# rbesenczi/newMSM

Hardware: AMD Instinct MI355X
Metric: label-cost evals/sec (higher is better)
Workload: dtype f64; 1 GPU; pairwise sulc (D=1) unary label-cost table, ico6 data grid / ico4 control grid, 19 labels, 48678 evals = 3187573 point samples per step (BASELINE config 2); kind=univariate, simmeasure=correlation, replicas=1

## Files before the change

include/msmhip.h:

```cpp
#ifndef MSMHIP_H
#define MSMHIP_H

#include <stddef.h>
#include <stdint.h>

#ifdef __cplusplus
extern "C" {
#endif

#define MSM_ABI_VERSION 11

#define MSM_OK 0
#define MSM_ERR_INVALID (-1)
#define MSM_ERR_HIP (-2)
#define MSM_ERR_OUTSIDE (-3)
#define MSM_ERR_NOTFOUND (-4)
#define MSM_ERR_NOGPU (-5)
#define MSM_ERR_STATE (-6)
#define MSM_ERR_CAPACITY (-7)
#define MSM_ERR_ROTATION (-8)

#define MSM_RAD 100.0
#define MSM_FOLDING 1e7

typedef struct msm_ctx msm_ctx;
typedef struct msm_mesh msm_mesh;
typedef struct msm_cost msm_cost;

int         msm_abi_version(void);
const char *msm_last_error(void);
int         msm_device_count(void);

int msm_icosphere_counts(int order, int32_t *V, int32_t *T);
int msm_icosphere(int order, double radius, double *xyz, int32_t *tri);
int msm_mesh_adjacency(const int32_t *tri, int32_t V, int32_t T, int32_t *nbr_ptr, int32_t *nbr, int32_t *tid_ptr, int32_t *tid);
int msm_vertex_areas(const double *xyz, const int32_t *tri, int32_t V, int32_t T, double *area);
int msm_resample_anatomy_grid(const double *cp_xyz, int32_t N, const int32_t *cp_tri, int32_t Tc, int32_t levels, double rad, int32_t *Va, int32_t *Ta,
                              double *axyz, int32_t *atri, int32_t *w_ptr, int32_t *w_cp, double *w_val, int32_t *face_ptr, int32_t *face_idx);
int msm_cp_spacings(const double *xyz, const int32_t *tri, int32_t V, int32_t T, double *maxsep, double *mvdmax);
int msm_label_sampling_grid(int sg_order, double max_dist, int abs_is_int, int32_t cap,
                            double *samples, int32_t *nsamples, double *barycentres, int32_t *nbarycentres);
int msm_rescale_sampling_grid(const double *samples, int32_t n, double *scale, double *labels);
int msm_rotation_matrix(const double ci[3], const double index[3], double R[9]);
int msm_cp_rotations(const double centre[3], const double *cp_xyz, int32_t N, double *rot);
int msm_estimate_triplets(const int32_t *tri, int32_t T, int32_t *triplets);
int msm_estimate_pairs(const int32_t *tri, int32_t V, int32_t T, int32_t *pairs);
int msm_octree_signature(const double *xyz, const int32_t *tri, int32_t V, int32_t T, int64_t stats[5], uint64_t *signature);
int msm_ray_table_check(const double *xyz, const int32_t *tri, int32_t V, int32_t T, int32_t nsamples, uint64_t seed, int64_t report[10]);

msm_ctx *msm_ctx_create(int device);
msm_ctx *msm_ctx_create_on_stream(int device, void *hip_stream);
void     msm_ctx_destroy(msm_ctx *ctx);
int      msm_ctx_synchronize(msm_ctx *ctx);
void    *msm_ctx_stream(msm_ctx *ctx);
void     msm_store_release_i64(int64_t *addr, int64_t value);
int64_t  msm_load_acquire_i64(const int64_t *addr);
int64_t  msm_min_acquire_i64(const int64_t *addr, int32_t n);
int      msm_ctx_wait_stream(msm_ctx *ctx, void *hip_stream);
int      msm_ctx_staging_stats(msm_ctx *ctx, int64_t out[4]);
int      msm_ctx_time_queries(msm_ctx *ctx, int enable);
int      msm_ctx_query_kernel_ms(msm_ctx *ctx, double *ms);
int      msm_query_lanes(int64_t n_queries);
void    *msm_host_alloc(msm_ctx *ctx, size_t bytes);
void     msm_host_free(msm_ctx *ctx, void *p);
int      msm_host_register(msm_ctx *ctx, void *p, size_t bytes);

msm_mesh *msm_mesh_create(msm_ctx *ctx, const double *xyz, int32_t V, const int32_t *tri, int32_t T);
void      msm_mesh_destroy(msm_mesh *m);
int       msm_mesh_update_coords(msm_mesh *m, const double *xyz);
int       msm_mesh_get_coords(msm_mesh *m, double *xyz);
int       msm_mesh_set_features(msm_mesh *m, const double *feat, int32_t D);
int       msm_mesh_sizes(const msm_mesh *m, int32_t *V, int32_t *T, int32_t *D);
int       msm_mesh_octree_stats(msm_mesh *m, int64_t stats[5]);
int       msm_mesh_octree_signature(msm_mesh *m, int64_t stats[5], uint64_t *signature);
int       msm_octree_forest_signatures(msm_ctx *ctx, const double *xyz, int32_t V, const int32_t *tri, int32_t T, int32_t B, uint64_t *signatures);
int       msm_mesh_prepare_search(msm_mesh *m, int wait, int32_t *ready);

#define MSM_WEIGHTS_PROJECTED 0
#define MSM_WEIGHTS_RAW 1
int msm_query_triangles(msm_mesh *target, const double *q_xyz, int32_t N, int32_t *tri_id, int32_t *v_id, double *w, int weight_mode);
int msm_closest_vertex(msm_mesh *target, const double *q_xyz, int32_t N, int32_t *v_id);
int msm_adaptive_barycentric_weights(msm_mesh *in_mesh, msm_mesh *new_mesh, const double *excl,
                                     int32_t *row_ptr, int32_t *col, double *val, int64_t cap, int64_t *nnz);
int msm_metric_resample(msm_mesh *in_mesh, const double *data, int32_t D, msm_mesh *new_mesh, const double *excl, double *out, double *excl_out);
int msm_sphere_project_warp(msm_mesh *from, const double *to_xyz, double *sphere_xyz, int32_t N);
int msm_mesh_sphere_project_warp(msm_mesh *sphere, msm_mesh *from, const double *to_xyz);
int msm_barycentric_coords_resample(msm_mesh *from, const double *coords_xyz, const double *q_xyz, int32_t N, double *out_xyz);
int msm_smooth_data(msm_mesh *orig, const double *data, int32_t D, msm_mesh *sphlow, double sigma, const double *excl, double *out, double *excl_out);
int msm_nearest_neighbour(msm_mesh *orig, const double *data, int32_t D, const double *q_xyz, int32_t N, const double *excl, double *out, double *excl_out);
int msm_create_exclusion(const double *data, int32_t D, int32_t V, double thrl, double thru, double *excl);

int msm_mesh_unfold(msm_mesh *m, double radius, int32_t *passes, int32_t *first_folded);
int msm_variance_normalise(double *data, int32_t D, int32_t V, const double *excl);
int msm_histogram_match(msm_ctx *ctx, int32_t n_src, int32_t D, int32_t Vs, const double *src, const double *src_excl, int32_t src_excl_rows,
                        int32_t Vt, const double *ref, const double *ref_excl, int32_t ref_excl_rows, double *out);
int msm_mcmc_optimise(const double *unary, const double *tcosts, const int32_t *triplets, int32_t N, int32_t L, int32_t T, double mcparam,
                      int32_t iters, uint64_t seed, int32_t *labeling);
int msm_fusion_icm_step(const double *unary2 , const double *quads , const int32_t *pairs , int32_t P,
                        const double *octets , const int32_t *triplets , int32_t T, int32_t N, int32_t max_passes,
                        int32_t *x );
int msm_pairwise_icm(const double *unary, const double *paircosts, const int32_t *pairs, int32_t N, int32_t L, int32_t P, int32_t max_passes, int32_t *labeling);
// ... 134 lines not shown
```

newmsm_amd/_lib.py:

```python
import ctypes as C
import os

_HERE = os.path.dirname(os.path.abspath(__file__))
LIB_PATH = os.environ.get("MSM_LIB_PATH") or os.path.join(_HERE, "libmsmhip.so")

c_dp = C.POINTER(C.c_double)
c_ip = C.POINTER(C.c_int32)
c_lp = C.POINTER(C.c_int64)

MSM_OK = 0
ERR_NAMES = {-1: "MSM_ERR_INVALID", -2: "MSM_ERR_HIP", -3: "MSM_ERR_OUTSIDE", -4: "MSM_ERR_NOTFOUND", -5: "MSM_ERR_NOGPU",
             -6: "MSM_ERR_STATE", -7: "MSM_ERR_CAPACITY", -8: "MSM_ERR_ROTATION"}


class MsmError(RuntimeError):

    def __init__(self, code, message):
        super().__init__("%s (%d): %s" % (ERR_NAMES.get(code, "MSM_ERR"), code, message))
        self.code = code


class GroupParams(C.Structure):
    _fields_ = [("simmeasure", C.c_int32), ("fixnan", C.c_int32), ("lambda_", C.c_double), ("mu", C.c_double),
                ("kappa", C.c_double), ("k_exp", C.c_double), ("rexp", C.c_double), ("range", C.c_double), ("percentile", C.c_double)]


class CostParams(C.Structure):
    _fields_ = [("kind", C.c_int32), ("simmeasure", C.c_int32), ("rmode", C.c_int32), ("reserved", C.c_int32),
                ("lambda_", C.c_double), ("mu", C.c_double), ("kappa", C.c_double), ("k_exp", C.c_double),
                ("rexp", C.c_double), ("range", C.c_double), ("percentile", C.c_double)]


_VP = C.c_void_p
SIGNATURES = {
    "msm_abi_version": (C.c_int, []),
    "msm_last_error": (C.c_char_p, []),
    "msm_device_count": (C.c_int, []),
    "msm_icosphere_counts": (C.c_int, [C.c_int, c_ip, c_ip]),
    "msm_icosphere": (C.c_int, [C.c_int, C.c_double, c_dp, c_ip]),
    "msm_mesh_adjacency": (C.c_int, [c_ip, C.c_int32, C.c_int32, c_ip, c_ip, c_ip, c_ip]),
    "msm_vertex_areas": (C.c_int, [c_dp, c_ip, C.c_int32, C.c_int32, c_dp]),
    "msm_resample_anatomy_grid": (C.c_int, [c_dp, C.c_int32, c_ip, C.c_int32, C.c_int32, C.c_double, c_ip, c_ip, c_dp, c_ip, c_ip, c_ip, c_dp, c_ip, c_ip]),
    "msm_cp_spacings": (C.c_int, [c_dp, c_ip, C.c_int32, C.c_int32, c_dp, c_dp]),
    "msm_label_sampling_grid": (C.c_int, [C.c_int, C.c_double, C.c_int, C.c_int32, c_dp, c_ip, c_dp, c_ip]),
    "msm_rescale_sampling_grid": (C.c_int, [c_dp, C.c_int32, c_dp, c_dp]),
    "msm_rotation_matrix": (C.c_int, [c_dp, c_dp, c_dp]),
    "msm_cp_rotations": (C.c_int, [c_dp, c_dp, C.c_int32, c_dp]),
    "msm_estimate_triplets": (C.c_int, [c_ip, C.c_int32, c_ip]),
    "msm_estimate_pairs": (C.c_int, [c_ip, C.c_int32, C.c_int32, c_ip]),
    "msm_octree_signature": (C.c_int, [c_dp, c_ip, C.c_int32, C.c_int32, C.POINTER(C.c_int64), C.POINTER(C.c_uint64)]),
    "msm_ray_table_check": (C.c_int, [c_dp, c_ip, C.c_int32, C.c_int32, C.c_int32, C.c_uint64, C.POINTER(C.c_int64)]),
    "msm_ctx_create": (_VP, [C.c_int]),
    "msm_ctx_create_on_stream": (_VP, [C.c_int, _VP]),
    "msm_ctx_destroy": (None, [_VP]),
    "msm_ctx_synchronize": (C.c_int, [_VP]),
    "msm_ctx_stream": (_VP, [_VP]),
    "msm_store_release_i64": (None, [_VP, C.c_int64]),
    "msm_load_acquire_i64": (C.c_int64, [_VP]),
    "msm_min_acquire_i64": (C.c_int64, [_VP, C.c_int32]),
    "msm_ctx_time_queries": (C.c_int, [_VP, C.c_int]),
    "msm_ctx_query_kernel_ms": (C.c_int, [_VP, c_dp]),
    "msm_query_lanes": (C.c_int, [C.c_int64]),
    "msm_group_context": (_VP, [_VP]),
    "msm_ctx_wait_stream": (C.c_int, [_VP, _VP]),
    "msm_ctx_staging_stats": (C.c_int, [_VP, C.POINTER(C.c_int64)]),
    "msm_host_alloc": (_VP, [_VP, C.c_size_t]),
    "msm_host_free": (None, [_VP, _VP]),
    "msm_host_register": (C.c_int, [_VP, _VP, C.c_size_t]),
    "msm_mesh_create": (_VP, [_VP, c_dp, C.c_int32, c_ip, C.c_int32]),
    "msm_mesh_destroy": (None, [_VP]),
    "msm_mesh_update_coords": (C.c_int, [_VP, c_dp]),
    "msm_mesh_get_coords": (C.c_int, [_VP, c_dp]),
    "msm_mesh_set_features": (C.c_int, [_VP, c_dp, C.c_int32]),
    "msm_mesh_sizes": (C.c_int, [_VP, c_ip, c_ip, c_ip]),
    "msm_mesh_octree_stats": (C.c_int, [_VP, c_lp]),
    "msm_mesh_octree_signature": (C.c_int, [_VP, c_lp, C.POINTER(C.c_uint64)]),
    "msm_octree_forest_signatures": (C.c_int, [_VP, c_dp, C.c_int32, c_ip, C.c_int32, C.c_int32, C.POINTER(C.c_uint64)]),
    "msm_query_triangles": (C.c_int, [_VP, c_dp, C.c_int32, c_ip, c_ip, c_dp, C.c_int]),
    "msm_closest_vertex": (C.c_int, [_VP, c_dp, C.c_int32, c_ip]),
    "msm_adaptive_barycentric_weights": (C.c_int, [_VP, _VP, c_dp, c_ip, c_ip, c_dp, C.c_int64, c_lp]),
    "msm_metric_resample": (C.c_int, [_VP, c_dp, C.c_int32, _VP, c_dp, c_dp, c_dp]),
    "msm_create_exclusion": (C.c_int, [c_dp, C.c_int32, C.c_int32, C.c_double, C.c_double, c_dp]),
    "msm_sphere_project_warp": (C.c_int, [_VP, c_dp, c_dp, C.c_int32]),
    "msm_mesh_sphere_project_warp": (C.c_int, [_VP, _VP, c_dp]),
    "msm_barycentric_coords_resample": (C.c_int, [_VP, c_dp, c_dp, C.c_int32, c_dp]),
    "msm_smooth_data": (C.c_int, [_VP, c_dp, C.c_int32, _VP, C.c_double, c_dp, c_dp, c_dp]),
    "msm_mesh_unfold": (C.c_int, [_VP, C.c_double, c_ip, c_ip]),
    "msm_mesh_prepare_search": (C.c_int, [_VP, C.c_int, c_ip]),
    "msm_variance_normalise": (C.c_int, [c_dp, C.c_int32, C.c_int32, c_dp]),
    "msm_histogram_match": (C.c_int, [_VP, C.c_int32, C.c_int32, C.c_int32, c_dp, c_dp, C.c_int32, C.c_int32, c_dp, c_dp, C.c_int32, c_dp]),
    "msm_mcmc_optimise": (C.c_int, [c_dp, c_dp, c_ip, C.c_int32, C.c_int32, C.c_int32, C.c_double, C.c_int32, C.c_uint64, c_ip]),
    "msm_fusion_icm_step": (C.c_int, [c_dp, c_dp, c_ip, C.c_int32, c_dp, c_ip, C.c_int32, C.c_int32, C.c_int32, c_ip]),
    "msm_pairwise_icm": (C.c_int, [c_dp, c_dp, c_ip, C.c_int32, C.c_int32, C.c_int32, C.c_int32, c_ip]),
    "msm_nearest_neighbour": (C.c_int, [_VP, c_dp, C.c_int32, c_dp, C.c_int32, c_dp, c_dp, c_dp]),
    "msm_cost_create": (_VP, [_VP, C.POINTER(CostParams)]),
    "msm_cost_destroy": (None, [_VP]),
    "msm_cost_set_meshes": (C.c_int, [_VP, _VP, _VP, _VP]),
    "msm_cost_set_anatomical": (C.c_int, [_VP, _VP, c_dp, c_dp, C.c_int32, c_ip, C.c_int32, c_ip, c_ip, c_dp, c_ip, c_ip]),
    "msm_cost_reset_source": (C.c_int, [_VP, _VP]),
    "msm_cost_reset_cpgrid": (C.c_int, [_VP, _VP]),
    "msm_cost_set_source_features": (C.c_int, [_VP, c_dp, C.c_int32]),
    "msm_cost_set_cfweight": (C.c_int, [_VP, c_dp, C.c_int32]),
    "msm_cost_set_spacings": (C.c_int, [_VP, c_dp, C.c_double]),
    "msm_cost_set_labels": (C.c_int, [_VP, c_dp, C.c_int32, c_dp]),
# ... 96 lines not shown
```

newmsm_amd/api.py:

```python
import ctypes as C

import numpy as np

from ._lib import CostParams, MsmError, c_dp, c_ip, c_lp, check, lib

WEIGHTS_PROJECTED = 0
WEIGHTS_RAW = 1
KINDS = dict(univariate=0, multivariate=1, patchwise=2, ho_univariate=3, ho_multivariate=4)


def _soa(points):
    a = np.ascontiguousarray(np.asarray(points, dtype=np.float64).reshape(-1, 3).T)
    return a, a.ctypes.data_as(c_dp)


def _aos(soa, n):
    return np.ascontiguousarray(np.asarray(soa).reshape(3, n).T)


def _tri_soa(tri):
    a = np.ascontiguousarray(np.asarray(tri, dtype=np.int32).reshape(-1, 3).T)
    return a, a.ctypes.data_as(c_ip)


# ... 51 lines not shown
    t, pt = _tri_soa(tri)
    ms = np.zeros(x.shape[1])
    mvd = C.c_double()
    check(lib().msm_cp_spacings(px, pt, x.shape[1], t.shape[1], ms.ctypes.data_as(c_dp), C.byref(mvd)))
    return ms, mvd.value


def label_sampling_grid(sg_order, max_dist, abs_is_int=False, cap=4096):
    s = np.zeros((3, cap))
    b = np.zeros((3, cap))
    ns, nb = C.c_int32(), C.c_int32()
    check(lib().msm_label_sampling_grid(sg_order, float(max_dist), int(abs_is_int), cap, s.ctypes.data_as(c_dp), C.byref(ns),
                                        b.ctypes.data_as(c_dp), C.byref(nb)))
    return np.ascontiguousarray(s[:, : ns.value].T), np.ascontiguousarray(b[:, : nb.value].T)


def rescale_sampling_grid(samples, scale):
    s, ps = _soa(samples)
    n = s.shape[1]
    out = np.zeros((3, n))
    sc = C.c_double(scale)
    check(lib().msm_rescale_sampling_grid(ps, n, C.byref(sc), out.ctypes.data_as(c_dp)))
    return np.ascontiguousarray(out.T), sc.value


def estimate_rotation_matrix(ci, index):
    R = np.zeros(9)
    check(lib().msm_rotation_matrix(_d(ci)[1], _d(index)[1], R.ctypes.data_as(c_dp)))
    return R.reshape(3, 3)


def cp_rotations(centre, cp_xyz):
    x, px = _soa(cp_xyz)
    rot = np.zeros((x.shape[1], 9))
    check(lib().msm_cp_rotations(_d(centre)[1], px, x.shape[1], rot.ctypes.data_as(c_dp)))
    return rot


def octree_signature(xyz, tri):
    x, px = _soa(xyz)
    t, pt = _tri_soa(tri)
    stats = (C.c_int64 * 5)()
    sig = C.c_uint64(0)
    check(lib().msm_octree_signature(px, pt, x.shape[1], t.shape[1], stats, C.byref(sig)))
    return dict(nodes=stats[0], leaves=stats[1], depth=stats[2], refs=stats[3], max_leaf=stats[4]), sig.value


def ray_table_check(xyz, tri, nsamples=20000, seed=1):
    x, px = _soa(xyz)
    t, pt = _tri_soa(tri)
    rep = (C.c_int64 * 10)()
    check(lib().msm_ray_table_check(px, pt, x.shape[1], t.shape[1], nsamples, seed, rep))
    return dict(points=rep[0], by_float=rep[1], by_fp64=rep[2], open=rep[3], violations=rep[4], unusable=rep[5], with_exclusions=rep[6], simple=bool(rep[7]), boxes_checked=rep[8], refused_by_boxes=rep[9])


def estimate_triplets(tri):
    t, pt = _tri_soa(tri)
    out = np.zeros((t.shape[1], 3), dtype=np.int32)
    check(lib().msm_estimate_triplets(pt, t.shape[1], out.ctypes.data_as(c_ip)))
    return out


def estimate_pairs(tri, V):
    t, pt = _tri_soa(tri)
    n = lib().msm_estimate_pairs(pt, V, t.shape[1], None)
    if n < 0:
        check(n)
    out = np.zeros((n, 2), dtype=np.int32)
    lib().msm_estimate_pairs(pt, V, t.shape[1], out.ctypes.data_as(c_ip))
    return out


class Context:

    def __init__(self, device=0, stream=None):
        L = lib()
        self.h = L.msm_ctx_create(device) if stream is None else L.msm_ctx_create_on_stream(device, C.c_void_p(stream))
        if not self.h:
            raise MsmError(-5, L.msm_last_error().decode())
        self.device = device

    def synchronize(self):
        check(lib().msm_ctx_synchronize(self.h))

    @property
    def stream(self):
        return lib().msm_ctx_stream(self.h)

    def wait_stream(self, hip_stream=None):
        check(lib().msm_ctx_wait_stream(self.h, C.c_void_p(hip_stream or 0)))

    def staging_stats(self):
        out = (C.c_int64 * 4)()
        check(lib().msm_ctx_staging_stats(self.h, out))
        return dict(blocks=int(out[0]), bytes=int(out[1]), allocated=int(out[2]), waits=int(out[3]))

    def host_array(self, shape, dtype=np.float64):
        n = int(np.prod(shape)) * np.dtype(dtype).itemsize
        p = lib().msm_host_alloc(self.h, max(n, 8))
        if not p:
            raise MsmError(-2, lib().msm_last_error().decode())
        buf = (C.c_char * max(n, 8)).from_address(p)
        return np.frombuffer(buf, dtype=dtype, count=int(np.prod(shape))).reshape(shape)

    def scratch_host_array(self, name, shape, dtype=np.float64):
        n = int(np.prod(shape)) * np.dtype(dtype).itemsize
# ... 767 lines not shown
```

newmsm_amd/csrc/internal.hpp:

```cpp
#pragma once

#include <hip/hip_runtime.h>

#include <cstdarg>
#include <cstdint>
#include <cstdio>
#include <functional>
#include <memory>
#include <mutex>
#include <string>
#include <vector>

#include "../../include/msmhip.h"
#include "devbuf.hpp"
#include "geom.hpp"

namespace msm {

void set_error(const char *fmt, ...);
int fail(int code, const char *fmt, ...);
void pool_trim();
size_t pool_idle_bytes();

#define MSM_HIP(call)                                                                                 \
    do {                                                                                              \
        hipError_t e_ = (call);                                                                       \
        if (e_ != hipSuccess) return msm::fail(MSM_ERR_HIP, "%s failed: %s", #call, hipGetErrorString(e_)); \
    } while (0)

#define MSM_TRY(call)               \
    do {                            \
        const int st_ = (call);     \
        if (st_) return st_;        \
    } while (0)

struct Adjacency {
    std::vector<int32_t> nbr_ptr, nbr, tid_ptr, tid;
};
void build_adjacency(const int32_t *tri , int V, int T, Adjacency &adj);
void icosphere_unit(int order, std::vector<double> &xyz_aos, std::vector<int32_t> &tri_aos);

struct alignas(128) TriRec {
    double v0[3], v1[3], v2[3];
    double s3[3];
    double d;
    int32_t id[3];
    int32_t tri;
    double reserved;
};
static_assert(sizeof(TriRec) == 128, "TriRec must be 128 bytes");

constexpr int kRayPieces = 9;

struct RayTable {
    bool simple = false;
    int G = 0;
    std::vector<int4> cell;
    std::vector<float4> edge;
    std::vector<int4> more;
    std::vector<int4> excl;
    double r2lo = 0, r2hi = 0;
};

struct FlatOctree {
    std::vector<int4> node;
    std::vector<double4> nodebox;
    int nmask_blocks = 0;
    std::vector<int32_t> parent;
    std::vector<int32_t> leaf_tri;
    std::vector<int32_t> grid;
    int grid_depth = 0;
    RayTable rays;
    int64_t stats[5] = {0, 0, 0, 0, 0};
    int dev_nnodes = 0, dev_entries = 0;
    int nnodes() const { return node.empty() ? dev_nnodes : (int)node.size(); }
    int nentries() const { return node.empty() ? dev_entries : (int)leaf_tri.size(); }
};
void build_octree(const double *xyz , const int32_t *tri , int V, int T, FlatOctree &out);
void build_ray_table(const double *xyz, const int32_t *tri, int V, int T, FlatOctree &tree);

struct DevTree {
    const int4 *node;
    const int32_t *parent;
    const int32_t *leaf_tri;
    const float4 *cone;
    const TriRec *rec;
    const int32_t *grid;
    int grid_depth;
    int simple;
    const unsigned long long *mask;
    int nnodes;
    int ray_G;
    const int4 *ray_cell;
    const float4 *ray_tri;
    const int4 *ray_more, *ray_excl;
    double ray_r2lo, ray_r2hi;
};

}

namespace msm {
struct Stager;
}

struct msm_ctx {
// ... 141 lines not shown
```

newmsm_amd/csrc/octree.cpp:

```cpp
#include <algorithm>
#include <atomic>
#include <cmath>
#include <chrono>
#include <cstdio>
#include <cstdlib>
#include <deque>
#include <unordered_map>

#include "host_parallel.hpp"
#include "internal.hpp"
#include "search_device.hpp"

#define TICK(name) do { if (std::getenv("MSMHIP_TIMING")) { auto now_ = std::chrono::steady_clock::now(); fprintf(stderr, "  %s %.1f ms\n", name, std::chrono::duration<double, std::milli>(now_ - tick_).count()); tick_ = now_; } } while (0)

namespace msm {

namespace {

struct BNode {
    int first_child = -1;
    int parent = -1;
    double b[3][3];
    std::vector<int32_t> tris;
    int total_size = 0, num_split = 0;
};

struct Builder {
    const double *xyz;
    const int32_t *tri;
    int V, T;
    std::deque<BNode> nodes;
    std::vector<double> box;
    const double *bxp = nullptr;

    void precompute_boxes() {
        box.resize((size_t)6 * T);
        bxp = box.data();
        parallel_chunks(T, T < 20000 ? 1 : std::min(host_workers(), 8), [&](int, int t0, int t1) {
            for (int t = t0; t < t1; ++t) {
                double *lo = &box[(size_t)6 * t], *hi = lo + 3;
                for (int a = 0; a < 3; ++a) lo[a] = hi[a] = xyz[a * V + tri[t]];
                for (int k = 1; k < 3; ++k)
                    for (int a = 0; a < 3; ++a) {
                        double c = xyz[a * V + tri[k * T + t]];
                        if (c < lo[a]) lo[a] = c;
                        if (c > hi[a]) hi[a] = c;
                    }
            }
        });
    }
    void aabb(int t, double lo[3], double hi[3]) const {
        const double *b = &bxp[(size_t)6 * t];
        for (int a = 0; a < 3; ++a) {
            lo[a] = b[a];
            hi[a] = b[3 + a];
        }
    }
    bool overlaps(int n, const double lo[3], const double hi[3]) const {
// ... 151 lines not shown
                bool opposite = false;
                for (int f = ptr[v]; f < ptr[v + 1]; ++f) opposite = opposite || head[f] == u;
                if (!opposite) ok.store(false, std::memory_order_relaxed);
            }
    });
    if (!ok.load()) return false;
    const long E = (long)3 * T / 2;
    if ((long)V - E + (long)T != 2) return false;
    return std::fabs(solid - 4.0 * M_PI) < 1e-6;
}

std::vector<double> safe_margins(const double *xyz, const int32_t *tri, int V, int T) {
    std::vector<double> band(T), lmax(T), vband(V, 0.0), margin(T);
    for (int t = 0; t < T; ++t) {
        const int id[3] = {tri[t], tri[T + t], tri[2 * T + t]};
        const V3 a = vtx(xyz, V, id[0]), b = vtx(xyz, V, id[1]), c = vtx(xyz, V, id[2]);
        const double la = norm(sub(b, c)), lb = norm(sub(a, c)), lc = norm(sub(a, b));
        const double area = 0.5 * norm(cross(sub(b, a), sub(c, a)));
        lmax[t] = std::fmax(la, std::fmax(lb, lc));
        const double lmin = std::fmin(la, std::fmin(lb, lc));
        band[t] = (area > 0 && lmin > 0) ? 1e-8 / (2 * area * lmin) : HUGE_VAL;
        if (!(band[t] == band[t])) band[t] = HUGE_VAL;
        for (int k = 0; k < 3; ++k) vband[id[k]] = std::fmax(vband[id[k]], band[t]);
    }
    for (int t = 0; t < T; ++t) {
        const double widest = std::fmax(vband[tri[t]], std::fmax(vband[tri[T + t]], vband[tri[2 * T + t]]));
        const double dist = std::fmax(1e-5 * lmax[t], 1e3 * widest);
        margin[t] = (std::isfinite(dist) && dist < 0.05 * lmax[t]) ? dist : HUGE_VAL;
    }
    return margin;
}

bool lacking_leaves(const FlatOctree &o, int n, const double lo[3], const double hi[3], int t, int cap, std::vector<int> &lack) {
    const double4 box = o.nodebox[n];
    const double blo[3] = {box.x, box.y, box.z};
    for (int a = 0; a < 3; ++a)
        if (hi[a] < blo[a] || lo[a] > blo[a] + box.w) return true;
    const int4 nd = o.node[n];
    if (nd.x < 0) {
        const int32_t *first = o.leaf_tri.data() + nd.y, *last = first + (-nd.x - 1);
        if (std::find(first, last, t) != last) return true;
        if ((int)lack.size() >= cap) return false;
        lack.push_back(n);
        return true;
    }
    for (int c = 0; c < 8; ++c)
        if (!lacking_leaves(o, nd.x + c, lo, hi, t, cap, lack)) return false;
    return true;
}

constexpr double kRayShell = 1e-4;
constexpr int kRayExclMax = 7;

}

void build_ray_table(const double *xyz, const int32_t *tri, int V, int T, FlatOctree &out) {
    auto tick_ = std::chrono::steady_clock::now();
    out.rays.G = 0;
    out.rays.cell.clear();
    out.rays.edge.clear();
    out.rays.simple = simple_star_surface(xyz, tri, V, T);
    const char *no_table = std::getenv("MSMHIP_DISABLE_RAYTABLE");
    if (!out.rays.simple || (no_table && no_table[0] == '1')) return;
    TICK("simple");
    const std::vector<double> margin = safe_margins(xyz, tri, V, T);
    TICK("margins");
    out.rays.edge.assign((size_t)3 * T, make_float4(0.f, 0.f, 0.f, 2.f));
    out.rays.excl.clear();
    out.rays.more.clear();
    out.rays.r2lo = (kRad - kRayShell) * (kRad - kRayShell);
    out.rays.r2hi = (kRad + kRayShell) * (kRad + kRayShell);
    std::vector<char> usable(T, 0);
    const int workers = host_workers();
    struct Chunk {
        std::vector<int4> excl;
        std::vector<int> owner;
    };
    std::vector<Chunk> chunk_out(4 * (size_t)workers + 1);
    parallel_chunks(T, workers, [&](int ci, int t_begin, int t_end) {
    std::vector<int> lack;
    Chunk &mine = chunk_out[ci];
    for (int t = t_begin; t < t_end; ++t) {
        const V3 v[3] = {vtx(xyz, V, tri[t]), vtx(xyz, V, tri[T + t]), vtx(xyz, V, tri[2 * T + t])};
        V3 s3;
        double pd;
        plane_of(v[0], v[1], v[2], s3, pd);
        const double rho = std::fabs(pd);
        if (!(margin[t] < HUGE_VAL) || !(rho > 0)) continue;
        const double thr = margin[t] / rho * (1 + 1e-6) + kRayFloatAllowance;
        if (!(thr < 0.1)) continue;
        V3 u[3];
        double cosmax = 1.0;
        bool ok = true;
        for (int k = 0; k < 3; ++k) {
            const double n = norm(v[k]);
            ok = ok && n > 0;
            u[k] = scale(v[k], 1.0 / n);
        }
        if (!ok) continue;
        for (int k = 0; k < 3; ++k) cosmax = std::fmin(cosmax, dot(u[k], u[(k + 1) % 3]));
        if (!(cosmax > 0.5)) continue;
        const double rlo = kRad - kRayShell, rhi = kRad + kRayShell;
        const double sag = rhi * (1 - std::sqrt(cosmax)) * (1 + 1e-9) + 1e-9;
        double lo[3] = {HUGE_VAL, HUGE_VAL, HUGE_VAL}, hi[3] = {-HUGE_VAL, -HUGE_VAL, -HUGE_VAL};
        for (int k = 0; k < 3; ++k) {
            const double c[3] = {u[k].x, u[k].y, u[k].z};
            for (int a = 0; a < 3; ++a) {
                lo[a] = std::fmin(lo[a], std::fmin(rlo * c[a], rhi * c[a]));
                hi[a] = std::fmax(hi[a], std::fmax(rlo * c[a], rhi * c[a]));
            }
        }
        for (int a = 0; a < 3; ++a) {
            lo[a] -= sag;
            hi[a] += sag;
        }
        lack.clear();
// ... 20 lines not shown
                const double4 nb = out.nodebox[lack[j]];
                const int d = out.node[lack[j]].w;
                if (d > 8) {
                    ok = false;
                    break;
                }
                const double size = 2 * kBounds / (double)(1 << d);
                const int ix = (int)std::lround((nb.x + kBounds) / size), iy = (int)std::lround((nb.y + kBounds) / size), iz = (int)std::lround((nb.z + kBounds) / size);
                bx[j] = (d << 24) | (ix << 16) | (iy << 8) | iz;
            }
            if (!ok) continue;
            excl = (int)mine.excl.size();
            mine.excl.push_back(make_int4(bx[0], bx[1], bx[2], (int)lack.size()));
            mine.owner.push_back(t);
            if (lack.size() > 3) {
                mine.excl.push_back(make_int4(bx[3], bx[4], bx[5], bx[6]));
                mine.owner.push_back(-1);
            }
        }
        e[1].w = __builtin_bit_cast(float, (int32_t)excl);
        e[2].w = 0.f;
        for (int k = 0; k < 3; ++k) out.rays.edge[(size_t)3 * t + k] = e[k];
        usable[t] = 1;
    }
    });
    for (const Chunk &c : chunk_out) {
        const int base = (int)out.rays.excl.size();
        for (size_t k = 0; k < c.excl.size(); ++k) {
            out.rays.excl.push_back(c.excl[k]);
            if (c.owner[k] >= 0) out.rays.edge[(size_t)3 * c.owner[k] + 1].w = __builtin_bit_cast(float, (int32_t)(base + (int)k));
        }
    }
    TICK("edges+robust");
    int G = 8;
    while (G < 512 && (double)G * G * 6 < 4.0 * T) G *= 2;
    out.rays.G = G;
    const size_t ncell = (size_t)6 * G * G;
    struct Cand {
        uint32_t cell;
        float score;
        int32_t tri;
    };
    std::vector<std::vector<Cand>> found_by(4 * (size_t)workers + 1);
    std::vector<int32_t> count(ncell + 1, 0);
    const double m = 1e-5;
    parallel_chunks(T, workers, [&](int ci, int t_begin, int t_end) {
    std::vector<Cand> &found = found_by[ci];
    found.reserve((size_t)(t_end - t_begin) * 8);
    for (int t = t_begin; t < t_end; ++t) {
        if (!usable[t]) continue;
        const V3 v[3] = {vtx(xyz, V, tri[t]), vtx(xyz, V, tri[T + t]), vtx(xyz, V, tri[2 * T + t])};
        const double ln[3] = {norm(v[0]), norm(v[1]), norm(v[2])};
        for (int f = 0; f < 6; ++f) {
            const int a = f >> 1, bb = (a + 1) % 3, cc = (a + 2) % 3;
            const double sgn = (f & 1) ? -1.0 : 1.0;
            double pu[3], pv[3];
            bool front = true;
            for (int k = 0; k < 3; ++k) {
                const double c[3] = {v[k].x, v[k].y, v[k].z};
                const double w = sgn * c[a];
                if (!(w > 0.05 * ln[k])) {
                    front = false;
                    break;
                }
                pu[k] = c[bb] / w;
                pv[k] = c[cc] / w;
            }
            if (!front) continue;
            const double umin = std::fmin(pu[0], std::fmin(pu[1], pu[2])) - m, umax = std::fmax(pu[0], std::fmax(pu[1], pu[2])) + m;
            const double vmin = std::fmin(pv[0], std::fmin(pv[1], pv[2])) - m, vmax = std::fmax(pv[0], std::fmax(pv[1], pv[2])) + m;
            if (umax < -1 || umin > 1 || vmax < -1 || vmin > 1) continue;
            auto cellof = [&](double x) { return std::max(0, std::min(G - 1, (int)std::floor((x + 1) * 0.5 * G))); };
            const int iu0 = cellof(umin), iu1 = cellof(umax), iv0 = cellof(vmin), iv1 = cellof(vmax);
            const double gu = (pu[0] + pu[1] + pu[2]) / 3, gv = (pv[0] + pv[1] + pv[2]) / 3;
            double ex[3], ey[3], ox[3], oy[3], sg[3];
            for (int k = 0; k < 3; ++k) {
                const int p = (k + 1) % 3, q = (k + 2) % 3;
                ex[k] = pu[q] - pu[p], ey[k] = pv[q] - pv[p], ox[k] = pu[p], oy[k] = pv[p];
                sg[k] = (ex[k] * (pv[k] - oy[k]) - ey[k] * (pu[k] - ox[k])) >= 0 ? 1.0 : -1.0;
            }
            for (int iu = iu0; iu <= iu1; ++iu)
                for (int iv = iv0; iv <= iv1; ++iv) {
                    const double x0 = -1 + 2.0 * iu / G - m, x1 = -1 + 2.0 * (iu + 1) / G + m;
                    const double y0 = -1 + 2.0 * iv / G - m, y1 = -1 + 2.0 * (iv + 1) / G + m;
                    bool sep = false;
                    for (int k = 0; k < 3 && !sep; ++k) {
                        auto E = [&](double x, double y) { return sg[k] * (ex[k] * (y - oy[k]) - ey[k] * (x - ox[k])); };
                        sep = E(x0, y0) < 0 && E(x1, y0) < 0 && E(x0, y1) < 0 && E(x1, y1) < 0;
                    }
                    if (sep) continue;
                    const double cu = 0.5 * (x0 + x1) - gu, cv = 0.5 * (y0 + y1) - gv;
                    const size_t cell = ((size_t)f * G + iu) * G + iv;
                    found.push_back(Cand{(uint32_t)cell, (float)(cu * cu + cv * cv), t});
                }
        }
    }
    });
    size_t nfound = 0;
    for (const auto &f : found_by) {
        nfound += f.size();
        for (const Cand &c : f) ++count[c.cell + 1];
    }
    TICK("raster");
    for (size_t c = 0; c < ncell; ++c) count[c + 1] += count[c];
    std::vector<Cand> cand(nfound);
    {
        std::vector<int32_t> fill(count.begin(), count.end() - 1);
        for (const auto &f : found_by)
            for (const Cand &c : f) cand[(size_t)fill[c.cell]++] = c;
    }
    TICK("bucket");
    out.rays.cell.assign(ncell, make_int4(-1, -1, -1, -1));
    parallel_chunks((int)ncell, workers, [&](int, int c_begin, int c_end) {
        for (int c = c_begin; c < c_end; ++c)
            std::sort(cand.data() + count[c], cand.data() + count[c + 1],
                      [](const Cand &x, const Cand &y) { return x.score < y.score || (x.score == y.score && x.tri < y.tri); });
    });
    for (size_t c = 0; c < ncell; ++c) {
        const Cand *first = cand.data() + count[c], *last = cand.data() + count[c + 1];
        int32_t *slot = &out.rays.cell[c].x;
        const int ncand = (int)(last - first);
        if (ncand <= 4) {
            for (int k = 0; k < ncand; ++k) slot[k] = first[k].tri;
        } else {
            for (int k = 0; k < 3; ++k) slot[k] = first[k].tri;
            slot[3] = -2 - (int)out.rays.more.size();
            int4 more = make_int4(-1, -1, -1, -1);
            int32_t *ms = &more.x;
            for (int k = 0; k < 4 && 3 + k < ncand; ++k) ms[k] = first[3 + k].tri;
            out.rays.more.push_back(more);
        }
    }
    TICK("cells");
}

namespace {

void build_top_down(Builder &b) {
    auto tick_ = std::chrono::steady_clock::now();
    std::vector<int32_t> all(b.T);
    for (int t = 0; t < b.T; ++t) all[t] = t;
    const int workers = host_workers();
    if (workers == 1 || b.T < 20000) {
        b.build_down(0, all);
        return;
    }
    struct Job {
        int node;
        std::vector<int32_t> list;
    };
    std::vector<Job> frontier, next;
    frontier.push_back(Job{0, std::move(all)});
    for (int level = 0; level < 2; ++level) {
        next.clear();
        std::vector<std::pair<int, int>> todo;
        for (size_t jn = 0; jn < frontier.size(); ++jn) {
            Job &j = frontier[jn];
            int total_size = 0, num_split = 0;
            bool splits = false;
            const int len = (int)j.list.size();
            for (int i = 0; i < len && !splits; ++i) {
                const double *bx = &b.bxp[(size_t)6 * j.list[i]];
                int split_size = 8;
                for (int d = 0; d < 3; ++d)
                    if ((bx[d] < b.nodes[j.node].b[d][1]) == (bx[3 + d] < b.nodes[j.node].b[d][1])) split_size >>= 1;
                total_size += split_size;
                if (split_size != 8) ++num_split;
                splits = i + 1 >= kMaxTriangles && num_split > 0 && total_size < 3 * (i + 1);
            }
            if (!splits) {
                b.nodes[j.node].tris = std::move(j.list);
                continue;
            }
            b.split(j.node);
            const int first = b.nodes[j.node].first_child;
            for (int c = 0; c < 8; ++c) {
                todo.push_back({(int)jn, (int)next.size()});
                next.push_back(Job{first + c, {}});
            }
        }
        parallel_for((int)todo.size() / 8, workers, [&](int k) {
            const Job &j = frontier[todo[8 * k].first];
            std::vector<int32_t> sub[8];
            b.distribute(j.node, j.list, sub);
            for (int c = 0; c < 8; ++c) next[todo[8 * k + c].second].list = std::move(sub[c]);
        });
// ... 210 lines not shown
            do p = mk(2 * rnd() - 1, 2 * rnd() - 1, 2 * rnd() - 1);
            while (!(norm(p) > 0.1 && norm(p) <= 1.0));
        } else {
            const int t = (int)(rnd() * T) % T, k = (int)(rnd() * 3) % 3;
            const V3 a = vert(t, k), b = vert(t, (k + 1) % 3), c = vert(t, (k + 2) % 3);
            const double along = kind == 3 ? (rnd() < 0.5 ? 0.0 : 1e-9 * rnd()) : rnd();
            const V3 on = mk(a.x + along * (b.x - a.x), a.y + along * (b.y - a.y), a.z + along * (b.z - a.z));
            const double off = (rnd() < 0.5 ? -1.0 : 1.0) * std::pow(10.0, -10.0 + 7.0 * rnd()) * (rnd() < 0.1 ? 0.0 : 1.0);
            p = mk(on.x + off * (c.x - on.x), on.y + off * (c.y - on.y), on.z + off * (c.z - on.z));
        }
        const double radius = kRad + (it % 7 == 0 ? (2 * rnd() - 1) * 0.9e-4 : 0.0);
        p = scale(normalized(p), radius);
        ++report[0];
        int n = 0;
        while (o.node[n].x >= 0) {
            const double4 b = o.nodebox[n];
            const double mx = (b.x + (b.x + b.w)) / 2.0, my = (b.y + (b.y + b.w)) / 2.0, mz = (b.z + (b.z + b.w)) / 2.0;
            n = o.node[n].x + 4 * (!(p.x < mx)) + 2 * (!(p.y < my)) + (!(p.z < mz));
        }
        hits.clear();
        for (int e = 0; e < -o.node[n].x - 1; ++e) {
            const int t = o.leaf_tri[o.node[n].y + e];
            const V3 a = vert(t, 0), b = vert(t, 1), c = vert(t, 2);
            if (point_in_triangle(project_point(p, a, b, c), a, b, c)) hits.push_back(t);
        }
        float fx, fy, fz;
        const int4 cell = ray_cell_of(dt, p, fx, fy, fz);
        int4 more = make_int4(cell.w, -1, -1, -1);
        if (cell.x >= 0 && cell.w < -1) more = o.rays.more[-2 - cell.w];
        const int cand[7] = {cell.x, cell.y, cell.z, more.x, more.y, more.z, more.w};
        const double pn = norm(p);
        bool by_float = false, by_fp64 = false, bad = false;
        for (int k = 0; k < 7 && cell.x >= 0; ++k) {
            const int t = cand[k];
            if (t < 0) break;
            const float4 e0 = o.rays.edge[3 * (size_t)t], e1 = o.rays.edge[3 * (size_t)t + 1], e2 = o.rays.edge[3 * (size_t)t + 2];
            float least;
            const int lvl = ray_accept_level(e0, e1, e2, fx, fy, fz, least);
            bool ok = lvl == 2;
            const bool fp64 = lvl == 1 && ray_accepts_fp64(vert(t, 0), vert(t, 1), vert(t, 2), p, pn, (double)e0.w - kRayFloatAllowance + 1e-12);
            ok = ok || fp64;
            if (ok && !ray_vouches(dt, e1, p)) ++report[9];
            if (!ok || !ray_vouches(dt, e1, p)) continue;
            (lvl == 2 ? by_float : by_fp64) = true;
            if (!(hits.size() == 1 && hits[0] == t)) bad = true;
        }
        if (bad) ++report[4];
        if (by_float) ++report[1];
        else if (by_fp64) ++report[2];
        else ++report[3];
    }
    return MSM_OK;
}
```

newmsm_amd/csrc/search_device.hpp:

```cpp
#pragma once

#include "internal.hpp"

namespace msm {

struct ScanState {
    int best;
    int have_d;
    double bestd;
};

__device__ __forceinline__ V3 rec_v0(const TriRec &r) { return mk(r.v0[0], r.v0[1], r.v0[2]); }
__device__ __forceinline__ V3 rec_v1(const TriRec &r) { return mk(r.v1[0], r.v1[1], r.v1[2]); }
__device__ __forceinline__ V3 rec_v2(const TriRec &r) { return mk(r.v2[0], r.v2[1], r.v2[2]); }

__device__ __forceinline__ bool inside_test(const TriRec &r, const V3 &p, V3 &mp) {
    mp = project_with_plane(p, mk(r.s3[0], r.s3[1], r.s3[2]), r.d);
    return point_in_triangle(mp, rec_v0(r), rec_v1(r), rec_v2(r));
}

MSM_HD int ray_clamp(int i, int hi) {
#ifdef __HIP_DEVICE_COMPILE__
    return max(0, min(hi, i));
#else
    return i < 0 ? 0 : (i > hi ? hi : i);
#endif
}
MSM_HD float ray_rsqrt(float x) {
#ifdef __HIP_DEVICE_COMPILE__
    return rsqrtf(x);
#else
    return 1.0f / sqrtf(x);
#endif
}
MSM_HD int4 ray_cell_of(const DevTree &T, const V3 &p, float &fx, float &fy, float &fz) {
    const double r2 = p.x * p.x + p.y * p.y + p.z * p.z;
    fx = fy = fz = 0.f;
    if (!(r2 >= T.ray_r2lo && r2 <= T.ray_r2hi)) return make_int4(-1, -1, -1, -1);
    const float qx = (float)p.x, qy = (float)p.y, qz = (float)p.z;
    const float inv = ray_rsqrt(qx * qx + qy * qy + qz * qz);
    fx = qx * inv, fy = qy * inv, fz = qz * inv;
    const float ax = fabsf(fx), ay = fabsf(fy), az = fabsf(fz);
    int face;
    float w, u, v;
    if (ax >= ay && ax >= az) {
        face = fx < 0.f ? 1 : 0, w = ax, u = fy, v = fz;
    } else if (ay >= az) {
        face = fy < 0.f ? 3 : 2, w = ay, u = fz, v = fx;
    } else {
        face = fz < 0.f ? 5 : 4, w = az, u = fx, v = fy;
    }
    const float iw = 1.0f / w, half = 0.5f * (float)T.ray_G;
    const int G = T.ray_G;
    const int iu = ray_clamp((int)((u * iw + 1.0f) * half), G - 1);
    const int iv = ray_clamp((int)((v * iw + 1.0f) * half), G - 1);
    return T.ray_cell[((size_t)face * G + iu) * G + iv];
}

MSM_HD bool ray_accepts(const float4 &e0, const float4 &e1, const float4 &e2, float fx, float fy, float fz) {
    const float d0 = __builtin_fmaf(e0.z, fz, __builtin_fmaf(e0.y, fy, e0.x * fx));
    const float d1 = __builtin_fmaf(e1.z, fz, __builtin_fmaf(e1.y, fy, e1.x * fx));
    const float d2 = __builtin_fmaf(e2.z, fz, __builtin_fmaf(e2.y, fy, e2.x * fx));
    return (int)(d0 >= e0.w) & (int)(d1 >= e0.w) & (int)(d2 >= e0.w);
}

MSM_HD int ray_accept_level(const float4 &e0, const float4 &e1, const float4 &e2, float fx, float fy, float fz, float &least) {
    const float d0 = __builtin_fmaf(e0.z, fz, __builtin_fmaf(e0.y, fy, e0.x * fx));
    const float d1 = __builtin_fmaf(e1.z, fz, __builtin_fmaf(e1.y, fy, e1.x * fx));
    const float d2 = __builtin_fmaf(e2.z, fz, __builtin_fmaf(e2.y, fy, e2.x * fx));
    least = fminf(d0, fminf(d1, d2));
    const float lo = e0.w - 6.5e-6f;
    if ((int)(d0 >= e0.w) & (int)(d1 >= e0.w) & (int)(d2 >= e0.w)) return 2;
    return (int)(d0 >= lo) & (int)(d1 >= lo) & (int)(d2 >= lo);
}
MSM_HD bool ray_accepts_fp64(const V3 &v0, const V3 &v1, const V3 &v2, const V3 &p, double pn, double thr) {
    bool ok = true;
#pragma unroll
    for (int k = 0; k < 3; ++k) {
        const V3 &a = k == 0 ? v1 : (k == 1 ? v2 : v0), &b = k == 0 ? v2 : (k == 1 ? v0 : v1), &c = k == 0 ? v0 : (k == 1 ? v1 : v2);
        const V3 n = cross(a, b);
        double val = dot(n, p);
        if (dot(n, c) < 0.0) val = -val;
        ok = ok && val >= thr * norm(n) * pn;
    }
    return ok;
}

MSM_HD bool ray_vouches(const DevTree &T, const float4 &e1, const V3 &p);

__device__ __forceinline__ double candidate_distance(const DevTree &T, int t, const V3 &p) {
    const TriRec &r = T.rec[t];
    V3 mp;
    inside_test(r, p, mp);
    return dist_to_point(mp, rec_v0(r), rec_v1(r), rec_v2(r));
}

__device__ __forceinline__ void exact_candidate(const DevTree &T, int t, const V3 &p, ScanState &s) {
    V3 mp;
    if (!inside_test(T.rec[t], p, mp)) return;
    if (s.best < 0) {
        s.best = t;
        s.have_d = 0;
        return;
    }
    if (!s.have_d) {
        s.bestd = candidate_distance(T, s.best, p);
        s.have_d = 1;
    }
    const double d = candidate_distance(T, t, p);
// ... 449 lines not shown
```

Before: 365.0 million evals/s.

## Pack per-subcell candidate hints into ray cell words to test likely triangle first

Each ray-table cell is split into a 3x3 grid of sub-cells. For each sub-cell, a 2-bit hint records which of the four listed candidate triangles contains the sub-cell centre. The hints go into the upper bits of the triangle id words, and the device lookup reorders the candidates so the hinted triangle is tried first. This aims to cut failed acceptance tests and fallbacks during point location. In exchange it adds id masking and reordering work per lookup, limits triangle ids to 26 bits, and adds a host check function.

Result: faster. 376.1 million evals/s (median of 6 runs) (+3.0%).

```diff
diff --git a/include/msmhip.h b/include/msmhip.h
--- a/include/msmhip.h
+++ b/include/msmhip.h
@@ -47,6 +47,8 @@
 int msm_estimate_pairs(const int32_t *tri, int32_t V, int32_t T, int32_t *pairs);
 int msm_octree_signature(const double *xyz, const int32_t *tri, int32_t V, int32_t T, int64_t stats[5], uint64_t *signature);
 int msm_ray_table_check(const double *xyz, const int32_t *tri, int32_t V, int32_t T, int32_t nsamples, uint64_t seed, int64_t report[10]);
+int msm_ray_hint_check(const double *xyz, const int32_t *tri, int32_t V, int32_t T, int32_t nsamples, uint64_t seed, int64_t report[8], int32_t *cells,
+                       int64_t cells_cap);
 
 msm_ctx *msm_ctx_create(int device);
 msm_ctx *msm_ctx_create_on_stream(int device, void *hip_stream);
diff --git a/newmsm_amd/_lib.py b/newmsm_amd/_lib.py
--- a/newmsm_amd/_lib.py
+++ b/newmsm_amd/_lib.py
@@ -50,6 +50,7 @@
     "msm_estimate_pairs": (C.c_int, [c_ip, C.c_int32, C.c_int32, c_ip]),
     "msm_octree_signature": (C.c_int, [c_dp, c_ip, C.c_int32, C.c_int32, C.POINTER(C.c_int64), C.POINTER(C.c_uint64)]),
     "msm_ray_table_check": (C.c_int, [c_dp, c_ip, C.c_int32, C.c_int32, C.c_int32, C.c_uint64, C.POINTER(C.c_int64)]),
+    "msm_ray_hint_check": (C.c_int, [c_dp, c_ip, C.c_int32, C.c_int32, C.c_int32, C.c_uint64, C.POINTER(C.c_int64), c_ip, C.c_int64]),
     "msm_ctx_create": (_VP, [C.c_int]),
     "msm_ctx_create_on_stream": (_VP, [C.c_int, _VP]),
     "msm_ctx_destroy": (None, [_VP]),
diff --git a/newmsm_amd/api.py b/newmsm_amd/api.py
--- a/newmsm_amd/api.py
+++ b/newmsm_amd/api.py
@@ -127,6 +127,18 @@
     rep = (C.c_int64 * 10)()
     check(lib().msm_ray_table_check(px, pt, x.shape[1], t.shape[1], nsamples, seed, rep))
     return dict(points=rep[0], by_float=rep[1], by_fp64=rep[2], open=rep[3], violations=rep[4], unusable=rep[5], with_exclusions=rep[6], simple=bool(rep[7]), boxes_checked=rep[8], refused_by_boxes=rep[9])
+
+
+def ray_hint_check(xyz, tri, nsamples=20000, seed=1, return_cells=False):
+    x, px = _soa(xyz)
+    t, pt = _tri_soa(tri)
+    rep = (C.c_int64 * 8)()
+    cells = np.zeros((6 * 512 * 512, 4), dtype=np.int32) if return_cells else None
+    check(lib().msm_ray_hint_check(px, pt, x.shape[1], t.shape[1], nsamples, seed, rep, cells.ctypes.data_as(c_ip) if return_cells else None, cells.size if return_cells else 0))
+    out = dict(points=rep[0], hinted=rep[1], unhinted=rep[2], listed=rep[3], cells_changed=rep[4], cells=rep[5], cells_with_more=rep[6], subcells=rep[7])
+    if return_cells:
+        out["cell_array"] = cells[: rep[5]].copy()
+    return out
 
 
 def estimate_triplets(tri):
diff --git a/newmsm_amd/csrc/internal.hpp b/newmsm_amd/csrc/internal.hpp
--- a/newmsm_amd/csrc/internal.hpp
+++ b/newmsm_amd/csrc/internal.hpp
@@ -51,6 +51,14 @@
 static_assert(sizeof(TriRec) == 128, "TriRec must be 128 bytes");
 
 constexpr int kRayPieces = 9;
+
+#ifndef MSM_RAY_HINT_K
+#define MSM_RAY_HINT_K 3
+#endif
+constexpr int kRayHintK = MSM_RAY_HINT_K;
+static_assert(kRayHintK >= 1 && kRayHintK <= 3, "two bits per sub-cell, three sub-cells per word, three words");
+constexpr int kRayIdBits = 26;
+constexpr int kRayMaxTris = 1 << (kRayIdBits - 1);
 
 struct RayTable {
     bool simple = false;
diff --git a/newmsm_amd/csrc/octree.cpp b/newmsm_amd/csrc/octree.cpp
--- a/newmsm_amd/csrc/octree.cpp
+++ b/newmsm_amd/csrc/octree.cpp
@@ -4,6 +4,7 @@
 #include <chrono>
 #include <cstdio>
 #include <cstdlib>
+#include <cstring>
 #include <deque>
 #include <unordered_map>
 
@@ -261,6 +262,31 @@
 constexpr double kRayShell = 1e-4;
 constexpr int kRayExclMax = 7;
 
+struct FaceTri {
+    double pu[3], pv[3], ex[3], ey[3], ox[3], oy[3], sg[3];
+    bool project(const V3 v[3], const double ln[3], int f) {
+        const int a = f >> 1, bb = (a + 1) % 3, cc = (a + 2) % 3;
+        const double sgn = (f & 1) ? -1.0 : 1.0;
+        for (int k = 0; k < 3; ++k) {
+            const double c[3] = {v[k].x, v[k].y, v[k].z};
+            const double w = sgn * c[a];
+            if (!(w > 0.05 * ln[k])) return false;
+            pu[k] = c[bb] / w;
+            pv[k] = c[cc] / w;
+        }
+        return true;
+    }
+    void edges() {
+        for (int k = 0; k < 3; ++k) {
+            const int p = (k + 1) % 3, q = (k + 2) % 3;
+            ex[k] = pu[q] - pu[p], ey[k] = pv[q] - pv[p], ox[k] = pu[p], oy[k] = pv[p];
+            sg[k] = (ex[k] * (pv[k] - oy[k]) - ey[k] * (pu[k] - ox[k])) >= 0 ? 1.0 : -1.0;
+        }
+    }
+    double E(int k, double x, double y) const { return sg[k] * (ex[k] * (y - oy[k]) - ey[k] * (x - ox[k])); }
+    bool holds(double x, double y) const { return E(0, x, y) >= 0 && E(1, x, y) >= 0 && E(2, x, y) >= 0; }
+};
+
 }
 
 void build_ray_table(const double *xyz, const int32_t *tri, int V, int T, FlatOctree &out) {
@@ -271,6 +297,7 @@
     out.rays.simple = simple_star_surface(xyz, tri, V, T);
     const char *no_table = std::getenv("MSMHIP_DISABLE_RAYTABLE");
     if (!out.rays.simple || (no_table && no_table[0] == '1')) return;
+    if (kRayHintK > 1 && T > kRayMaxTris) return;
     TICK("simple");
     const std::vector<double> margin = safe_margins(xyz, tri, V, T);
     TICK("margins");
@@ -397,42 +424,23 @@
         const V3 v[3] = {vtx(xyz, V, tri[t]), vtx(xyz, V, tri[T + t]), vtx(xyz, V, tri[2 * T + t])};
         const double ln[3] = {norm(v[0]), norm(v[1]), norm(v[2])};
         for (int f = 0; f < 6; ++f) {
-            const int a = f >> 1, bb = (a + 1) % 3, cc = (a + 2) % 3;
-            const double sgn = (f & 1) ? -1.0 : 1.0;
-            double pu[3], pv[3];
-            bool front = true;
-            for (int k = 0; k < 3; ++k) {
-                const double c[3] = {v[k].x, v[k].y, v[k].z};
-                const double w = sgn * c[a];
-                if (!(w > 0.05 * ln[k])) {
-                    front = false;
-                    break;
-                }
-                pu[k] = c[bb] / w;
-                pv[k] = c[cc] / w;
-            }
-            if (!front) continue;
+            FaceTri ft;
+            if (!ft.project(v, ln, f)) continue;
+            const double *pu = ft.pu, *pv = ft.pv;
             const double umin = std::fmin(pu[0], std::fmin(pu[1], pu[2])) - m, umax = std::fmax(pu[0], std::fmax(pu[1], pu[2])) + m;
             const double vmin = std::fmin(pv[0], std::fmin(pv[1], pv[2])) - m, vmax = std::fmax(pv[0], std::fmax(pv[1], pv[2])) + m;
             if (umax < -1 || umin > 1 || vmax < -1 || vmin > 1) continue;
             auto cellof = [&](double x) { return std::max(0, std::min(G - 1, (int)std::floor((x + 1) * 0.5 * G))); };
             const int iu0 = cellof(umin), iu1 = cellof(umax), iv0 = cellof(vmin), iv1 = cellof(vmax);
             const double gu = (pu[0] + pu[1] + pu[2]) / 3, gv = (pv[0] + pv[1] + pv[2]) / 3;
-            double ex[3], ey[3], ox[3], oy[3], sg[3];
-            for (int k = 0; k < 3; ++k) {
-                const int p = (k + 1) % 3, q = (k + 2) % 3;
-                ex[k] = pu[q] - pu[p], ey[k] = pv[q] - pv[p], ox[k] = pu[p], oy[k] = pv[p];
-                sg[k] = (ex[k] * (pv[k] - oy[k]) - ey[k] * (pu[k] - ox[k])) >= 0 ? 1.0 : -1.0;
-            }
+            ft.edges();
             for (int iu = iu0; iu <= iu1; ++iu)
                 for (int iv = iv0; iv <= iv1; ++iv) {
                     const double x0 = -1 + 2.0 * iu / G - m, x1 = -1 + 2.0 * (iu + 1) / G + m;
                     const double y0 = -1 + 2.0 * iv / G - m, y1 = -1 + 2.0 * (iv + 1) / G + m;
                     bool sep = false;
-                    for (int k = 0; k < 3 && !sep; ++k) {
-                        auto E = [&](double x, double y) { return sg[k] * (ex[k] * (y - oy[k]) - ey[k] * (x - ox[k])); };
-                        sep = E(x0, y0) < 0 && E(x1, y0) < 0 && E(x0, y1) < 0 && E(x1, y1) < 0;
-                    }
+                    for (int k = 0; k < 3 && !sep; ++k)
+                        sep = ft.E(k, x0, y0) < 0 && ft.E(k, x1, y0) < 0 && ft.E(k, x0, y1) < 0 && ft.E(k, x1, y1) < 0;
                     if (sep) continue;
                     const double cu = 0.5 * (x0 + x1) - gu, cv = 0.5 * (y0 + y1) - gv;
                     const size_t cell = ((size_t)f * G + iu) * G + iv;
@@ -477,6 +485,49 @@
         }
     }
     TICK("cells");
+    if (kRayHintK > 1) {
+        parallel_chunks((int)ncell, workers, [&](int, int c_begin, int c_end) {
+            for (int c = c_begin; c < c_end; ++c) {
+                int4 &cell = out.rays.cell[c];
+                const int f = c / (G * G), iu = (c / G) % G, iv = c % G;
+                const int ids[4] = {cell.x, cell.y, cell.z, cell.w};
+                FaceTri ft[4];
+                int state[4] = {0, 0, 0, 0};
+                auto holds = [&](int j, double x, double y) {
+                    if (state[j] == 0) {
+                        const int t = ids[j];
+                        state[j] = -1;
+                        if (t >= 0) {
+                            const V3 v[3] = {vtx(xyz, V, tri[t]), vtx(xyz, V, tri[T + t]), vtx(xyz, V, tri[2 * (size_t)T + t])};
+                            const double ln[3] = {0.0, 0.0, 0.0};
+                            if (ft[j].project(v, ln, f)) {
+                                ft[j].edges();
+                                state[j] = 1;
+                            }
+                        }
+                    }
+                    return state[j] > 0 && ft[j].holds(x, y);
+                };
+                uint32_t bits[3] = {0u, 0u, 0u};
+                for (int su = 0; su < kRayHintK && ids[1] >= 0; ++su)
+                    for (int sv = 0; sv < kRayHintK; ++sv) {
+                        const double x = -1 + 2.0 * (iu + (su + 0.5) / kRayHintK) / G, y = -1 + 2.0 * (iv + (sv + 0.5) / kRayHintK) / G;
+                        uint32_t h = 0;
+                        for (int j = 0; j < 4; ++j)
+                            if (holds(j, x, y)) {
+                                h = (uint32_t)j;
+                                break;
+                            }
+                        bits[su] |= h << (kRayIdBits + 2 * sv);
+                    }
+                const uint32_t idmask = (1u << kRayIdBits) - 1u;
+                cell.x = (int32_t)(((uint32_t)cell.x & idmask) | bits[0]);
+                cell.y = (int32_t)(((uint32_t)cell.y & idmask) | bits[1]);
+                cell.z = (int32_t)(((uint32_t)cell.z & idmask) | bits[2]);
+            }
+        });
+        TICK("hints");
+    }
 }
 
 namespace {
@@ -793,3 +844,88 @@
     }
     return MSM_OK;
 }
+
+extern "C" int msm_ray_hint_check(const double *xyz, const int32_t *tri, int32_t V, int32_t T, int32_t nsamples, uint64_t seed, int64_t report[8], int32_t *cells,
+                                  int64_t cells_cap) {
+    using namespace msm;
+    if (!xyz || !tri || !report || V <= 0 || T <= 0 || nsamples < 0) return fail(MSM_ERR_INVALID, "msm_ray_hint_check: bad arguments");
+    for (int64_t i = 0; i < 3 * (int64_t)T; ++i)
+        if (tri[i] < 0 || tri[i] >= V) return fail(MSM_ERR_INVALID, "msm_ray_hint_check: triangle vertex id %d out of range [0,%d)", tri[i], V);
+    FlatOctree o;
+    build_octree(xyz, tri, V, T, o);
+    build_ray_table(xyz, tri, V, T, o);
+    for (int k = 0; k < 8; ++k) report[k] = 0;
+    report[7] = kRayHintK;
+    if (o.rays.G <= 0) return MSM_OK;
+    const size_t ncell = o.rays.cell.size();
+    report[5] = (int64_t)ncell;
+    if (cells) {
+        if (cells_cap < 4 * (int64_t)ncell) return fail(MSM_ERR_INVALID, "msm_ray_hint_check: room for %lld words, the cells have %lld", (long long)cells_cap, (long long)(4 * ncell));
+        std::memcpy(cells, o.rays.cell.data(), ncell * sizeof(int4));
+    }
+    for (size_t c = 0; c < ncell; ++c) {
+        const int4 raw = o.rays.cell[c], ids = ray_cell_ids(raw);
+        if (ids.x >= 0 && ids.w < -1) ++report[6];
+        const int stored[4] = {ids.x, ids.y, ids.z, ids.w};
+        bool same = true;
+        for (int k = 0; k < 4; ++k) same = same && stored[k] < T && (stored[k] >= -1 || (k == 3 && -2 - stored[k] < (int)o.rays.more.size()));
+        for (int su = 0; su < kRayHintK && same; ++su)
+            for (int sv = 0; sv < kRayHintK && same; ++sv) {
+                const int h = ray_cell_hint(raw, su, sv);
+                const int4 d = ray_cell_first(raw, h);
+                const int got[4] = {d.x, d.y, d.z, d.w};
+                same = got[0] == stored[h] && (stored[0] < 0 || got[0] >= 0);
+                for (int k = 0, j = 1; k < 4; ++k)
+                    if (k != h) same = same && got[j++] == stored[k];
+            }
+        if (!same) ++report[4];
+    }
+    DevTree dt{};
+    dt.ray_G = o.rays.G;
+    dt.ray_cell = o.rays.cell.data();
+    dt.ray_more = o.rays.more.data();
+    dt.ray_excl = o.rays.excl.data();
+    dt.ray_r2lo = o.rays.r2lo, dt.ray_r2hi = o.rays.r2hi;
+    uint64_t rs = seed * 6364136223846793005ull + 1442695040888963407ull;
+    auto rnd = [&]() {
+        rs = rs * 6364136223846793005ull + 1442695040888963407ull;
+        return (double)(rs >> 11) * (1.0 / 9007199254740992.0);
+    };
+    auto vert = [&](int t, int k) { return vtx(xyz, V, tri[(size_t)k * T + t]); };
+    for (int it = 0; it < nsamples; ++it) {
+        V3 p;
+        do p = mk(2 * rnd() - 1, 2 * rnd() - 1, 2 * rnd() - 1);
+        while (!(norm(p) > 0.1 && norm(p) <= 1.0));
+        p = scale(normalized(p), kRad);
+        ++report[0];
+        int n = 0;
+        while (o.node[n].x >= 0) {
+            const double4 b = o.nodebox[n];
+            const double mx = (b.x + (b.x + b.w)) / 2.0, my = (b.y + (b.y + b.w)) / 2.0, mz = (b.z + (b.z + b.w)) / 2.0;
+            n = o.node[n].x + 4 * (!(p.x < mx)) + 2 * (!(p.y < my)) + (!(p.z < mz));
+        }
+        int answer = -1, nhits = 0;
+        for (int e = 0; e < -o.node[n].x - 1; ++e) {
+            const int t = o.leaf_tri[o.node[n].y + e];
+            const V3 a = vert(t, 0), b = vert(t, 1), c = vert(t, 2);
+            if (point_in_triangle(project_point(p, a, b, c), a, b, c)) answer = t, ++nhits;
+        }
+        if (nhits != 1) continue;
+        float fx, fy, fz;
+        size_t at;
+        int su, sv;
+        if (!ray_cell_at(dt, p, fx, fy, fz, at, su, sv)) continue;
+        const int4 first = ray_cell_of(dt, p, fx, fy, fz), ids = ray_cell_ids(o.rays.cell[at]);
+        if (first.x == answer) ++report[1];
+        if (ids.x == answer) ++report[2];
+        int4 more = make_int4(ids.w, -1, -1, -1);
+        if (ids.x >= 0 && ids.w < -1) more = o.rays.more[-2 - ids.w];
+        const int list[7] = {ids.x, ids.y, ids.z, more.x, more.y, more.z, more.w};
+        for (int k = 0; k < 7; ++k)
+            if (list[k] == answer) {
+                ++report[3];
+                break;
+            }
+    }
+    return MSM_OK;
+}
diff --git a/newmsm_amd/csrc/search_device.hpp b/newmsm_amd/csrc/search_device.hpp
--- a/newmsm_amd/csrc/search_device.hpp
+++ b/newmsm_amd/csrc/search_device.hpp
@@ -33,10 +33,25 @@
     return 1.0f / sqrtf(x);
 #endif
 }
-MSM_HD int4 ray_cell_of(const DevTree &T, const V3 &p, float &fx, float &fy, float &fz) {
+MSM_HD int ray_cell_id(int word) { return (int)((unsigned)word << (32 - kRayIdBits)) >> (32 - kRayIdBits); }
+MSM_HD int4 ray_cell_ids(const int4 &raw) {
+    if (kRayHintK == 1) return raw;
+    return make_int4(ray_cell_id(raw.x), ray_cell_id(raw.y), ray_cell_id(raw.z), raw.w);
+}
+MSM_HD int ray_cell_hint(const int4 &raw, int su, int sv) {
+    if (kRayHintK == 1) return 0;
+    const unsigned word = (unsigned)(su == 0 ? raw.x : (su == 1 ? raw.y : raw.z));
+    return (int)((word >> (kRayIdBits + 2 * sv)) & 3u);
+}
+MSM_HD int4 ray_cell_first(const int4 &raw, int h) {
+    const int4 c = ray_cell_ids(raw);
+    if (kRayHintK == 1) return c;
+    return make_int4(h == 0 ? c.x : (h == 1 ? c.y : (h == 2 ? c.z : c.w)), h >= 1 ? c.x : c.y, h >= 2 ? c.y : c.z, h == 3 ? c.z : c.w);
+}
+MSM_HD bool ray_cell_at(const DevTree &T, const V3 &p, float &fx, float &fy, float &fz, size_t &at, int &su, int &sv) {
     const double r2 = p.x * p.x + p.y * p.y + p.z * p.z;
     fx = fy = fz = 0.f;
-    if (!(r2 >= T.ray_r2lo && r2 <= T.ray_r2hi)) return make_int4(-1, -1, -1, -1);
+    if (!(r2 >= T.ray_r2lo && r2 <= T.ray_r2hi)) return false;
     const float qx = (float)p.x, qy = (float)p.y, qz = (float)p.z;
     const float inv = ray_rsqrt(qx * qx + qy * qy + qz * qz);
     fx = qx * inv, fy = qy * inv, fz = qz * inv;
@@ -52,9 +67,29 @@
     }
     const float iw = 1.0f / w, half = 0.5f * (float)T.ray_G;
     const int G = T.ray_G;
-    const int iu = ray_clamp((int)((u * iw + 1.0f) * half), G - 1);
-    const int iv = ray_clamp((int)((v * iw + 1.0f) * half), G - 1);
-    return T.ray_cell[((size_t)face * G + iu) * G + iv];
+    const float gu = (u * iw + 1.0f) * half, gv = (v * iw + 1.0f) * half;
+    const int iu = ray_clamp((int)gu, G - 1);
+    const int iv = ray_clamp((int)gv, G - 1);
+    su = ray_clamp((int)((gu - (float)iu) * (float)kRayHintK), kRayHintK - 1);
+    sv = ray_clamp((int)((gv - (float)iv) * (float)kRayHintK), kRayHintK - 1);
+    at = ((size_t)face * G + iu) * G + iv;
+    return true;
+}
+MSM_HD int4 ray_cell_of(const DevTree &T, const V3 &p, float &fx, float &fy, float &fz) {
+    size_t at;
+    int su, sv;
+    if (!ray_cell_at(T, p, fx, fy, fz, at, su, sv)) return make_int4(-1, -1, -1, -1);
+    const int4 raw = T.ray_cell[at];
+    int4 c = ray_cell_first(raw, ray_cell_hint(raw, su, sv));
+#ifdef __HIP_DEVICE_COMPILE__
+    if (kRayHintK > 1) {
+        typedef int v4i __attribute__((ext_vector_type(4)));
+        v4i q = {c.x, c.y, c.z, c.w};
+        asm volatile("" : "+v"(q));
+        c = make_int4(q.x, q.y, q.z, q.w);
+    }
+#endif
+    return c;
 }
 
 MSM_HD bool ray_accepts(const float4 &e0, const float4 &e1, const float4 &e2, float fx, float fy, float fz) {
```
